# wjwei-handsome/wgatools

Measured on AMD Instinct MI355X. Metric: paf_cigar_ops_per_s (paf2maf+stat), higher is better.
Workload: dtype u8

## Files before the change

wgatools_amd/csrc/wga_kernels_k2s.h:

```cpp
#ifndef WGA_KERNELS_K2S_H
#define WGA_KERNELS_K2S_H

#include "wga_kernels.h"

#define WGA_S_FIFO 320u
#define WGA_S_MAX_JOB_TILES 32u
#define WGA_S_U 4u
#define WGA_S_WAVE_BYTES ((WGA_S_FIFO + 4u) * 8u + 1024u + 1024u + 256u + 272u + 16u)
#ifndef WGA_AUTO_LONG_VARIANT
#define WGA_AUTO_LONG_VARIANT 3
#endif

__global__ __launch_bounds__(256) void k_pseudo_rec_desc(u32 n, const wga_class_sums* sums, const u8* strand_neg, const u64* q_src_off,
                                                         const u64* q_src_len, const u64* skip, const u64* dst_off, const u64* op_off,
                                                         u64 q_fa_bytes, wga_rec_desc* out, u8* tile_flag) {
  const u32 r = blockIdx.x * 256u + threadIdx.x;
  if (r >= n) return;
  const wga_class_sums cs = sums[r];
  wga_rec_desc d;
  d.t_row_off = 0;
  d.q_row_off = dst_off[r] - skip[r];
  d.t_src_off = 0;
  d.t_src_len = skip[r];
  d.q_src_off = q_src_off ? q_src_off[r] : 0ull;
  d.q_src_len = q_src_len ? q_src_len[r] : 0ull;
  d.I_total = cs.i + cs.s;
  d.D_total = cs.d;
  d.L = cs.mx + cs.d;
  const bool clean = !q_src_len || d.q_src_len == cs.mx + cs.i + cs.s;
  const bool inside = !q_src_off || (d.q_src_off >= 32ull && d.q_src_off + d.q_src_len + 32ull <= q_fa_bytes);
  d.neg = (strand_neg[r] != 0 ? 1u : 0u) | (clean ? 0u : 8u);
  out[r] = d;
  if (clean && inside) return;
  const u64 a = op_off[r], b = op_off[r + 1];
  if (b <= a) return;
  for (u64 t = a / WGA_TILE; t <= (b - 1) / WGA_TILE; t++) tile_flag[t] = 1;
}

__device__ __forceinline__ u32 comp4s(u32 x, u32* bad) {
  const u32 sel = x & 0x07070707u;
  const u32 fold = byte_perm(0x474EFF54u, 0x43FF41FFu, sel);
  const u32 comp = byte_perm(0x434E0D41u, 0x47FF54FFu, sel);
  *bad = (x & 0xDFDFDFDFu) ^ fold;
  return comp | (x & 0x20202020u);
}

#define WGA_S_NOINLINE __forceinline__
__device__ WGA_S_NOINLINE void stream_store_bytes(u8* p, u32 o0, u32 o1, u32 o2, u32 o3, int lo, int hi) {
#pragma clang loop vectorize(disable) unroll(disable)
  for (int j = lo; j < hi; j++) {
    const u32 wj = j < 4 ? o0 : j < 8 ? o1 : j < 12 ? o2 : o3;
    p[j] = (u8)(wj >> (8 * (j & 3)));
  }
}
__device__ WGA_S_NOINLINE void stream_report_bad(u64* bad_base_pos, u32 b0, u32 b1, u32 b2, u32 b3, int lo, int hi, u32 Cl,
                                                 i64 Kseg, const u32* fifo, u32 k, u32 nf, u32 adj) {
#pragma clang loop vectorize(disable) unroll(disable)
  for (int j = lo; j < hi; j++) {
    const u32 bw = j < 4 ? b0 : j < 8 ? b1 : j < 12 ? b2 : b3;
    if (((bw >> (8 * (j & 3))) & 0xFFu) == 0u) continue;
    const u32 cj = Cl + (u32)j;
    u32 ad = adj;
    if (fifo) {
      u32 i = k - 1u;
      while (i + 1u < nf && (int)(fifo[2u * (i + 1u)] - cj) <= 0) i++;
      ad = fifo[2u * (i + 1u) + 1u];
    }
    atomicMin(bad_base_pos, (u64)((i64)(u64)(cj - ad) + Kseg));
  }
}

#define WGA_S_PSEUDO 2
#define WGA_S_SYMBOL 3
template <int MODE>
__device__ __forceinline__ u32 stream_glen(u32 c0, u32 c1) {
  return MODE == WGA_S_SYMBOL ? (c1 >> 1) - (c0 >> 1) : MODE == WGA_S_PSEUDO ? ((int)(c1 - c0) > 0 ? c1 - c0 : 0u) : c1 - c0;
}
__device__ __forceinline__ u32 stream_symbol(u32 cu) { return (cu & 1u) ? 0x2D2D2D2Du : 0x30303030u; }
template <int MODE>
__device__ __forceinline__ void stream_row(const ExpandArgs& a, u8* const lds, const u32 lane, const u64 job, const u64 t0,
                                           const u64 t1) {
  const u32 skipm = WGA_RO32(a.job_skip + job);
  u32* const s_fifo = (u32*)lds;
  u32x4_a16* const s_P = (u32x4_a16*)(s_fifo + 2u * (WGA_S_FIFO + 4u));
  u32* const s_q = (u32*)(s_P + 64);
  u32* const s_T = s_q + 256;
  u32x4_a16* const s_lm = (u32x4_a16*)(s_T + 64);
  u64* const s_k = (u64*)(s_lm + 17);
  if (lane < 17u) {
    u32x4_a16 m;
    for (int d = 0; d < 4; d++) m[d] = bytemask(0, (int)lane - 4 * d);
    s_lm[lane] = m;
  }
  constexpr bool QROW = MODE != 0;
  constexpr bool TCOORD = MODE >= WGA_S_PSEUDO;
  constexpr bool SYM = MODE == WGA_S_SYMBOL;
  constexpr u32 COL_MASK = TCOORD ? 0x585u : 0x787u;
  constexpr u32 GAP_MASK = MODE == 0 ? 0x202u : SYM ? 0x504u : 0x404u;
  constexpr u32 SKIP_MASK = MODE == WGA_S_PSEUDO ? 0x212u : 0u;
  const u8* const fa = QROW ? a.q_fa : a.t_fa;
  const u64 fa_bytes = QROW ? a.q_fa_bytes : a.t_fa_bytes;
  const u64 job_lo = t0 * WGA_TILE;
  const u32 q_end = WGA_UNI32((u32)((t1 * WGA_TILE < a.n_ops ? t1 * WGA_TILE : a.n_ops) - job_lo));
  const BufRsrc obuf = buf_make(a.ops + job_lo, (u32)(((a.n_ops - job_lo) < 0x3FFFFFFFull ? (a.n_ops - job_lo) : 0x3FFFFFFFull) * 4ull));

  u32 C_known = 0, cum_known = 0;
  u32 nf = 1;
  u32 e0 = 1;
  u32 pos = 0;
  u32 q = 0;
  u32 q_lo = 0, q_hi = 0;
  u32 rec = 0, re = 0;
  u8* dst_seg = nullptr;
  BufRsrc sbuf = buf_make(fa, 0u);
  u32 S32 = 0;
  bool rc = false;
  bool live = false;
  bool bnd = false;
  bool fin = false;
  u32 C_b = 0, cum_b = 0;
  u32 C_min = 0;
  u64 t = t0;
  u32 ow[4] = {0, 0, 0, 0}, xl0 = 0, xg0 = 0;
  u32 own[4] = {0, 0, 0, 0};

  auto fifo_dedupe = [&]() {
    WGA_WAVE_SYNC();
    u32 n_new = nf;
    if (lane == 0u) {
      u32 w = e0;
      for (u32 r = e0; r < nf; r++) {
        const u32 gs = s_fifo[2u * r], cu = s_fifo[2u * r + 1u];
        const bool dup = w > e0 && s_fifo[2u * (w - 1u)] == gs && (int)(cu - s_fifo[2u * (w - 1u) + 1u]) <= 0 &&
                         (int)(s_fifo[2u * (r + 1u) + 1u] - cu) <= 0;
        if (!dup) {
          s_fifo[2u * w] = gs;
          s_fifo[2u * w + 1u] = cu;
          w++;
        }
      }
      for (u32 k = 0; k < 3u; k++) {
        s_fifo[2u * (w + k)] = s_fifo[2u * (nf + k)];
        s_fifo[2u * (w + k) + 1u] = s_fifo[2u * (nf + k) + 1u];
      }
      n_new = w;
    }
    nf = wave_get_u32(n_new, 0);
    WGA_WAVE_SYNC();
  };

  for (;;) {
    {
      const u32 lim = bnd ? C_b : C_known;
      const bool all = bnd || fin;
      while ((int)(lim - pos) > 0) {
        if (TCOORD && (int)(C_min - pos) > 0) {
          const u32 to = (int)(lim - C_min) > 0 ? C_min : lim;
          u32 c;
          do {
            const u32 idx = e0 + lane < nf ? e0 + lane : nf;
            c = (u32)__popcll(__ballot(idx < nf && (int)(s_fifo[2u * idx] - to) < 0));
            e0 += c;
          } while (c == 64u);
          pos = to;
          continue;
        }
        u8* const A = dst_seg + pos;
        const u32 mis = (u32)(u64)A & 1023u;
        u8* const B = A - mis;
        const u32 room = WGA_S_U * 1024u - mis;
        if (!all && (lim - pos) < room) break;
        const u32 Cs = pos;
        u32 Ce = (lim - pos) < room ? lim : pos + room;
        const u32 Cl0 = Cs - mis;
        if (e0 + 255u < nf) {
          const u32 g255 = WGA_UNI32(s_fifo[2u * (e0 + 255u)]);
          if ((int)(g255 - Ce) < 0) Ce = Cl0 + ((g255 - Cl0) & ~15u);
          if (MODE == WGA_S_PSEUDO && (int)(Ce - Cs) < 16) {
            fifo_dedupe();
            continue;
          }
        }

        s_T[lane] = 0u;
        WGA_WAVE_SYNC();
        u32 nE = 0;
        {
          u32 base = e0, c;
          do {
            const u32 idx = base + lane < nf ? base + lane : nf;
            const u32 gsr = s_fifo[2u * idx] - Cl0;
            const bool in = gsr < Ce - Cl0;
            c = (u32)__popcll(__ballot(in));
            if (in) atomicAdd(&s_T[(gsr >> 4) & 63u], 1u << (8u * (gsr >> 10)));
            base += c;
            nE += c;
          } while (c == 64u);
        }
        WGA_WAVE_SYNC();
        const u32 tw = s_T[lane];
        WGA_WAVE_SYNC();
        const u32 tinc = wave_incl_scan_u32(tw);
        const u32 texc = tinc - tw;
        const u32 ttot = wave_last_u32(tinc);

        u32 kbase = e0;
        u32 qn = 0, rpk = 0, cls = 0;
        u32 adjv[WGA_S_U];
        const u32 wsp = Ce - Cs - 16u, asp = Ce - Cs + 15u;
        const bool any16 = (Ce - Cs) >= 16u;
        u32 qcum = 0;
#pragma unroll
        for (u32 u = 0; u < WGA_S_U; u++) {
          const u32 cnt = (tw >> (8u * u)) & 255u;
          const u32 k = kbase + ((texc >> (8u * u)) & 255u);
          kbase += (ttot >> (8u * u)) & 255u;
          const u32 Cl = Cl0 + 1024u * u + 16u * lane;
          const bool whole = any16 && (Cl - Cs) <= wsp, active = (Cl + 15u - Cs) < asp;
          const u32x4_a1 fe = *(const u32x4_a1*)(s_fifo + 2u * (k - 1u));
          const int rel0 = (int)(fe[0] + stream_glen<MODE>(fe[1], fe[3]) - Cl);
          const bool quiet = whole && cnt == 0u;
          const bool plain = quiet && rel0 <= 0;
          const bool dashes = quiet && rel0 >= 16;
          const bool flagged = active && !(plain || dashes);
          adjv[u] = fe[3];
          cls |= ((plain ? 1u : 0u) | (dashes ? 2u : 0u) | (flagged ? 4u : 0u) | (SYM ? (fe[1] & 1u) << 3 : 0u)) << (4u * u);
          const u64 m = __ballot(flagged);
          if (flagged) {
            const u32 r = qn + lane_rank(m, lane);
            s_q[r & 255u] = (k << 8) | (u << 6) | lane;
            rpk |= (r & 255u) << (8u * u);
          }
          qcum |= (qn > 255u ? 255u : qn) << (8u * u);
          qn += (u32)__popcll(m);
        }
        if (qn > 64u) {
          u32 keep = 1u;
#pragma unroll
          for (u32 u = 2; u <= WGA_S_U; u++) {
            const u32 upto = u == WGA_S_U ? qn : (qcum >> (8u * u)) & 255u;
            const bool sat = u < WGA_S_U && ((qcum >> (8u * u)) & 255u) == 255u;
            if (upto <= 64u && !sat) keep = u;
          }
          const u32 Cn = Cl0 + 1024u * keep;
          if ((int)(Cn - Ce) < 0) Ce = Cn;
          qn = keep == WGA_S_U ? qn : (qcum >> (8u * keep)) & 255u;
          nE = 0;
#pragma unroll
          for (u32 u = 0; u < WGA_S_U; u++)
            if (u < keep) nE += (ttot >> (8u * u)) & 255u;
        }
        const BufRsrc dbuf = buf_make(B, WGA_S_U * 1024u);

        WGA_WAVE_SYNC();
        if (lane < qn) {
          const u32 ent = s_q[lane];
          const u32 k = ent >> 8, Cl = Cl0 + 16u * (ent & 255u);
          int lo = (int)(Cs - Cl), hi = (int)(Ce - Cl);
          lo = lo < 0 ? 0 : (lo > 16 ? 16 : lo);
          hi = hi > 16 ? 16 : (hi < 0 ? 0 : hi);
          const u32x4_a1 ea = *(const u32x4_a1*)(s_fifo + 2u * (k - 1u));
          const u32x4_a1 eb = *(const u32x4_a1*)(s_fifo + 2u * (k + 1u));
          const u32 gs0 = ea[0], cu0 = ea[1], gs1 = ea[2], cu1 = ea[3], gs2 = eb[0], cu2 = eb[1];
          int a1 = (int)(gs0 + stream_glen<MODE>(cu0, cu1) - Cl);
          a1 = a1 < lo ? lo : (a1 > hi ? hi : a1);
          int b1 = (int)(gs1 - Cl);
          b1 = b1 < a1 ? a1 : (b1 > hi ? hi : b1);
          const u32 gl1 = stream_glen<MODE>(cu1, cu2);
          int e1 = gl1 >= 16u ? 16 : b1 + (int)gl1;
          e1 = e1 > hi ? hi : e1;
          bool more = (int)(gs2 - Cl) < hi;
          u32 W0[4], W1[4];
          if (!SYM) {
            buf_load16(sbuf, b1 > a1 ? (rc ? S32 - Cl + cu1 : S32 + Cl - cu1) : WGA_BUF_OOB, W0);
            buf_load16(sbuf, hi > e1 ? (rc ? S32 - Cl + cu2 : S32 + Cl - cu2) : WGA_BUF_OOB, W1);
          }
          const u32x4_a16 La = s_lm[a1], Lb = s_lm[b1], Le = s_lm[e1];
          u32 o[4], bad[4] = {0u, 0u, 0u, 0u};
#pragma unroll
          for (int d = 0; d < 4; d++) {
            if (SYM) {
              o[d] = bfi_b32(La[d], stream_symbol(cu0), bfi_b32(Le[d] & ~Lb[d], stream_symbol(cu1), 0x31313131u));
              continue;
            }
            u32 cp;
            if (rc)
              cp = comp4s(bfi_b32(Lb[d], bswap32(W0[3 - d]), bswap32(W1[3 - d])), &bad[d]);
            else
              cp = bfi_b32(Lb[d], W0[d], W1[d]);
            const u32 md = La[d] | (Le[d] & ~Lb[d]);
            o[d] = bfi_b32(md, 0x2D2D2D2Du, cp);
            bad[d] &= ~md;
          }
          u32 ie = k + 1u;
          while (more) {
            const u32 gsi = s_fifo[2u * ie], cui = s_fifo[2u * ie + 1u], gsn = s_fifo[2u * ie + 2u], cun = s_fifo[2u * ie + 3u];
            const int b = (int)(gsi - Cl);
            const u32 len = stream_glen<MODE>(cui, cun);
            const int e = len >= (u32)(hi - b) ? hi : b + (int)len;
            u32 W[4];
            if (SYM)
              W[0] = W[1] = W[2] = W[3] = 0x31313131u;
            else
              buf_load16(sbuf, rc ? S32 - Cl + cun : S32 + Cl - cun, W);
            const u32x4_a16 Mb = s_lm[b], Me = s_lm[e];
#pragma unroll
            for (int d = 0; d < 4; d++) {
              u32 x = W[d], bw = 0u;
              if (rc) x = comp4s(bswap32(W[3 - d]), &bw);
              if (SYM)
                o[d] = bfi_b32(Mb[d], o[d], bfi_b32(Me[d], stream_symbol(cui), x));
              else
                o[d] = bfi_b32(Mb[d], o[d], bfi_b32(Me[d], 0x2D2D2D2Du, x));
              bad[d] = (bad[d] & Mb[d]) | (bw & ~Me[d]);
            }
            ie++;
            more = (int)(gsn - Cl) < hi;
          }
          if (rc && (bad[0] | bad[1] | bad[2] | bad[3]) != 0u)
            stream_report_bad((u64*)&a.diag[rec].bad_base_pos, bad[0], bad[1], bad[2], bad[3], lo, hi, Cl, (i64)s_k[0], s_fifo, k, nf, 0u);
          const u32x4_a16 ov = {o[0], o[1], o[2], o[3]};
          s_P[lane] = ov;
        }
        WGA_WAVE_SYNC();

        u32 dat[WGA_S_U][4];
        const u32 wsp2 = Ce - Cs - 16u;
#pragma unroll
        for (u32 u = 0; u < WGA_S_U; u++) {
          const u32 Cl = Cl0 + 1024u * u + 16u * lane;
          const u32 c = (cls >> (4u * u)) & 15u;
          if (SYM) {
            dat[u][0] = dat[u][1] = dat[u][2] = dat[u][3] = (c & 2u) ? ((c & 8u) ? 0x2D2D2D2Du : 0x30303030u) : 0x31313131u;
            continue;
          }
          dat[u][0] = dat[u][1] = dat[u][2] = dat[u][3] = (c & 2u) ? 0x2D2D2D2Du : 0u;
          if ((c & 1u) && (int)(Cl - Ce) < 0) buf_load16(sbuf, rc ? S32 - Cl + adjv[u] : S32 + Cl - adjv[u], dat[u]);
        }
        if (rc) {
#pragma unroll
          for (u32 u = 0; u < WGA_S_U; u++) {
            u32 bad[4], x[4];
#pragma unroll
            for (int d = 0; d < 4; d++) x[d] = comp4s(bswap32(dat[u][3 - d]), &bad[d]);
#pragma unroll
            for (int d = 0; d < 4; d++) dat[u][d] = x[d];
            const u32 Cl = Cl0 + 1024u * u + 16u * lane;
            const bool pb = ((cls >> (4u * u)) & 1u) != 0u && (int)(Cl - Ce) < 0 && (bad[0] | bad[1] | bad[2] | bad[3]) != 0u;
            if (__ballot(pb)) {
              if (pb)
                stream_report_bad((u64*)&a.diag[rec].bad_base_pos, bad[0], bad[1], bad[2], bad[3], 0, 16, Cl, (i64)s_k[0], nullptr, 0u, 0u,
                                  adjv[u]);
            }
          }
        }
#pragma unroll
        for (u32 u = 0; u < WGA_S_U; u++) {
          const u32 Cl = Cl0 + 1024u * u + 16u * lane;
          const bool queued = ((cls >> (4u * u)) & 4u) != 0u && (int)(Cl - Ce) < 0;
          if (queued) {
            const u32x4_a16 pv = s_P[(rpk >> (8u * u)) & 255u];
            dat[u][0] = pv[0];
            dat[u][1] = pv[1];
            dat[u][2] = pv[2];
            dat[u][3] = pv[3];
          }
          const bool whole = (Ce - Cs) >= 16u && (Cl - Cs) <= wsp2;
          buf_store16_stream(dbuf, whole ? 1024u * u + 16u * lane : WGA_BUF_OOB, dat[u]);
          if (queued && !whole) {
            int lo = (int)(Cs - Cl), hi = (int)(Ce - Cl);
            lo = lo < 0 ? 0 : lo;
            hi = hi > 16 ? 16 : hi;
            stream_store_bytes(B + 1024u * u + lane * 16u, dat[u][0], dat[u][1], dat[u][2], dat[u][3], lo, hi);
          }
        }
        WGA_WAVE_SYNC();
        e0 += nE;
        pos = Ce;
      }
      fin = false;
    }

    if (bnd || !live) {
      const bool sw = bnd;
      u64 row_off, src_off, src_len, x_a, sb;
      bool neg;
      u32 C_a, cum_a;
      if (bnd) {
        const u64 bnd_op = job_lo + re;
        u64 ren, skip = 0;
        wga_u64x2 src;
        u32 negw;
        do {
          rec++;
          const wga_rec_desc* const rd = a.recs + rec;
          ren = WGA_RO64(a.op_off + rec + 1);
          row_off = WGA_RO64(QROW ? &rd->q_row_off : &rd->t_row_off);
          src = wga_ro16(QROW ? &rd->q_src_off : &rd->t_src_off);
          negw = WGA_RO32((const u32*)&rd->neg);
          if (TCOORD) skip = WGA_RO64(&rd->t_src_len);
          WGA_RO_HERE4(ren, row_off, src.x, src.y);
          WGA_RO_HERE2(negw, skip);
        } while (ren <= bnd_op);
        re = ren - job_lo > (u64)q_end ? q_end : (u32)(ren - job_lo);
        src_off = src.x;
        src_len = src.y;
        neg = (negw & 1u) != 0u;
        x_a = 0;
        sb = 0;
        C_a = C_b;
        cum_a = cum_b;
        if (TCOORD)
          C_min = C_a + (u32)(skip < 0x40000000ull ? skip : 0x40000000ull);
      } else {
        while (t < t1 && ((skipm >> (u32)(t - t0)) & 1u)) t++;
        if (t >= t1) break;
        const wga_tile_desc* const td = a.tdesc + t;
        const u64 tile_start = t * WGA_TILE;
        q = (u32)(tile_start - job_lo);
        WGA_WAVE_SYNC();
        C_known = cum_known = 0u;
        pos = 0u;
        nf = 1u;
        e0 = 1u;
        if (lane < 4u) {
          s_fifo[2u * lane] = 0u;
          s_fifo[2u * lane + 1u] = 0u;
        }
        rec = WGA_RO32(&td->rec);
        const u64 ren = WGA_RO64(&td->re), rs = WGA_RO64(&td->rs);
        const u64 d_mx = WGA_RO64(&td->b_mx), d_i = WGA_RO64(&td->b_i), d_d = WGA_RO64(&td->b_d);
        row_off = WGA_RO64(QROW ? &td->q_row_off : &td->t_row_off);
        src_off = WGA_RO64(QROW ? &td->q_src_off : &td->t_src_off);
        src_len = WGA_RO64(QROW ? &td->q_src_len : &td->t_src_len);
        neg = (WGA_RO32(&td->neg) & 1u) != 0u;
        const u64 skip = TCOORD ? WGA_RO64(&td->t_src_len) : 0ull;
        re = ren - job_lo > (u64)q_end ? q_end : (u32)(ren - job_lo);
        const bool cont = rs < tile_start;
        const u64 b_mx = cont ? d_mx : 0ull, b_i = cont ? d_i : 0ull, b_d = cont ? d_d : 0ull;
        x_a = TCOORD ? b_mx + b_d : b_mx + b_i + b_d;
        sb = QROW ? b_mx + b_i : b_mx + b_d;
        C_a = cum_a = 0u;
        if (TCOORD) {
          const u64 ahead = skip > x_a ? skip - x_a : 0ull;
          C_min = (u32)(ahead < 0x40000000ull ? ahead : 0x40000000ull);
        }
        buf_load16(obuf, q * 4u + lane * 16u, own);
        live = true;
      }
      dst_seg = (u8*)((u64)a.out + row_off + x_a - (u64)C_a);
      rc = QROW && !SYM && neg;
      const u32 adv = C_a - cum_a;
      u64 base;
      if (rc) {
        const u64 top = src_off + src_len;
        const u64 hiB = top > sb ? top - sb : 0ull;
        base = hiB > 0x60000000ull ? hiB - 0x60000000ull : 0ull;
        S32 = (u32)(top - base) - 16u - (u32)sb + adv;
      } else {
        const u64 loB = src_off + sb;
        base = loB > 64ull ? loB - 64ull : 0ull;
        S32 = (u32)(loB - base) - adv;
      }
      base = base > fa_bytes ? fa_bytes : base;
      {
        const u64 left = fa_bytes - base;
        sbuf = buf_make(fa + base, left > 0xFFFFFFF0ull ? 0xFFFFFFF0u : (u32)left);
      }
      if (lane == 0u) s_k[0] = (u64)((i64)sb - (i64)(u64)adv);
      WGA_WAVE_SYNC();
      bnd = false;
      if (sw && re < q_hi) {
        const u32 kb = re - q_lo, e = kb & 3u;
        u32 vl = xl0, vg = xg0;
#pragma unroll
        for (u32 i = 0; i < 3u; i++) {
          const bool valid = q_lo + 4u * lane + i < q_hi && i < e;
          const u32 len = valid ? ow[i] >> 4 : 0u, code = ow[i] & 15u;
          vl += len & bit_mask(COL_MASK, code);
          vg += (len & bit_mask(GAP_MASK, code)) - (len & bit_mask(SKIP_MASK, code));
        }
        C_b = wave_get_u32_dyn(vl, kb >> 2);
        cum_b = wave_get_u32_dyn(vg, kb >> 2);
        bnd = true;
      }
      continue;
    }

    if (q >= q_end) {
      if (pos != C_known) {
        fin = true;
        continue;
      }
      break;
    }
    if ((q & (WGA_TILE - 1u)) == 0u) {
      t = (job_lo + q) / WGA_TILE;
      if ((skipm >> (u32)(t - t0)) & 1u) {
        if (pos != C_known) {
          fin = true;
          continue;
        }
        live = false;
        t++;
        continue;
      }
    }
    if (e0 > 1u) {
      const u32 from = e0 - 1u, count = nf + 3u - from;
      for (u32 i0 = 0; i0 < count; i0 += 64u) {
        const u32 i = i0 + lane;
        u64 v = 0;
        if (i < count) v = *(const u64*)(s_fifo + 2u * (from + i));
        WGA_WAVE_SYNC();
        if (i < count) *(u64*)(s_fifo + 2u * i) = v;
        WGA_WAVE_SYNC();
      }
      nf -= from;
      e0 = 1u;
    }
    if (nf + 256u > WGA_S_FIFO) {
      fin = true;
      if (pos != C_known) continue;
      fin = false;
      if (MODE == WGA_S_PSEUDO) {
        fifo_dedupe();
        if (nf + 256u > WGA_S_FIFO) break;
      }
    }
    q_lo = q;
    q_hi = q + 256u < q_end ? q + 256u : q_end;
    q = q_hi;
    ow[0] = own[0], ow[1] = own[1], ow[2] = own[2], ow[3] = own[3];
    buf_load16(obuf, q_hi < q_end ? q_hi * 4u + lane * 16u : WGA_BUF_OOB, own);
    u32 l[4], g[4], sl = 0, sg = 0, sc = 0;
#pragma unroll
    for (int e = 0; e < 4; e++) {
      const bool valid = q_lo + 4u * lane + (u32)e < q_hi;
      const u32 len = valid ? ow[e] >> 4 : 0u, code = ow[e] & 15u;
      l[e] = len & bit_mask(COL_MASK, code);
      g[e] = (len & bit_mask(GAP_MASK, code)) - (len & bit_mask(SKIP_MASK, code));
      sl += l[e];
      sg += g[e];
      sc += g[e] != 0u ? 1u : 0u;
    }
    const u32 il = wave_incl_scan_u32(sl), ig = wave_incl_scan_u32(sg), ic = wave_incl_scan_u32(sc);
    xl0 = C_known + il - sl;
    xg0 = cum_known + ig - sg;
    {
      u32 xl = xl0, xg = xg0, xc = nf + ic - sc;
#pragma unroll
      for (int e = 0; e < 4; e++) {
        if (g[e] != 0u) {
          s_fifo[2u * xc] = xl;
          s_fifo[2u * xc + 1u] = SYM ? (xg << 1) | (bit_mask(0x404u, ow[e] & 15u) & 1u) : xg;
          xc++;
          xg += g[e];
        }
        xl += l[e];
      }
    }
    C_known += wave_last_u32(il);
    cum_known += wave_last_u32(ig);
    nf += wave_last_u32(ic);
    if (lane < 3u) {
      s_fifo[2u * (nf + lane)] = C_known;
      s_fifo[2u * (nf + lane) + 1u] = SYM ? cum_known << 1 : cum_known;
    }
    WGA_WAVE_SYNC();
    if (re < q_hi) {
      const u32 kb = re - q_lo, e = kb & 3u;
      u32 vl = xl0, vg = xg0;
#pragma unroll
      for (u32 i = 0; i < 3u; i++) {
        const bool valid = q_lo + 4u * lane + i < q_hi && i < e;
        const u32 len = valid ? ow[i] >> 4 : 0u, code = ow[i] & 15u;
        vl += len & bit_mask(COL_MASK, code);
        vg += (len & bit_mask(GAP_MASK, code)) - (len & bit_mask(SKIP_MASK, code));
      }
      C_b = wave_get_u32_dyn(vl, kb >> 2);
      cum_b = wave_get_u32_dyn(vg, kb >> 2);
      bnd = true;
    }
  }
}

__device__ __forceinline__ u64 xcd_job_of_block() {
  const u32 nb = gridDim.x, b = blockIdx.x, x = b & 7u, q = nb >> 3, r = nb & 7u;
  return (u64)(x * q + (x < r ? x : r) + (b >> 3));
}

__device__ __forceinline__ void expand_stream(const ExpandArgs& a) {
  __shared__ u32x4_a16 s_mem[2u * WGA_S_WAVE_BYTES / 16u];
  const u32 lane = threadIdx.x & 63u, wave = WGA_WAVE_ID(threadIdx.x);
  const u64 nt = (a.n_ops + WGA_TILE - 1) / WGA_TILE;
  const u64 job = xcd_job_of_block();
  const u64 t0 = job * a.job_tiles;
  if (t0 >= nt) return;
  const u64 t1 = t0 + a.job_tiles < nt ? t0 + a.job_tiles : nt;
  u8* const lds = (u8*)s_mem + wave * WGA_S_WAVE_BYTES;
  if (wave == 0u)
    stream_row<0>(a, lds, lane, job, t0, t1);
  else
    stream_row<1>(a, lds, lane, job, t0, t1);
}
template <int MODE>
__device__ __forceinline__ void pseudo_stream(const ExpandArgs& a) {
  __shared__ u32x4_a16 s_mem[2u * WGA_S_WAVE_BYTES / 16u];
  const u32 lane = threadIdx.x & 63u, wave = WGA_WAVE_ID(threadIdx.x);
  const u64 nt = (a.n_ops + WGA_TILE - 1) / WGA_TILE;
  const u64 job = 2u * xcd_job_of_block() + wave;
  const u64 t0 = job * a.job_tiles;
  if (t0 >= nt) return;
  const u64 t1 = t0 + a.job_tiles < nt ? t0 + a.job_tiles : nt;
  stream_row<MODE>(a, (u8*)s_mem + wave * WGA_S_WAVE_BYTES, lane, job, t0, t1);
}
#ifndef WGA_S_WAVES_PER_SIMD
#define WGA_S_WAVES_PER_SIMD 5
#endif
__global__ __launch_bounds__(128, WGA_S_WAVES_PER_SIMD) void k_paf2maf_expand_s(ExpandArgs a) { expand_stream(a); }
__global__ __launch_bounds__(128, WGA_S_WAVES_PER_SIMD) void k_pafpseudo_stream(ExpandArgs a) { pseudo_stream<WGA_S_PSEUDO>(a); }
#ifndef WGA_S_SYM_WAVES
#define WGA_S_SYM_WAVES 5
#endif
__global__ __launch_bounds__(128, WGA_S_SYM_WAVES) void k_pafpseudo_stream_sym(ExpandArgs a) { pseudo_stream<WGA_S_SYMBOL>(a); }

#endif
```

Before: 80.08 billion.

## Double-buffer CIGAR op prefetch through LDS via direct DMA loads

Replaces the register-held next-chunk op prefetch with a two-slot LDS ring filled by LDS-direct DMA loads, falling back to buffer loads at the tail. Boundary computation now reads the op words from LDS rather than from per-lane registers. The aim is to lower register pressure and overlap op fetch with the sequence-copy work, and explicit vm_wait calls order the data. In exchange it uses 2 KB more LDS per wave, which may lower occupancy, and adds waits that can serialize on outstanding sequence loads.

```diff
diff --git a/wgatools_amd/csrc/wga_kernels_k2s.h b/wgatools_amd/csrc/wga_kernels_k2s.h
--- a/wgatools_amd/csrc/wga_kernels_k2s.h
+++ b/wgatools_amd/csrc/wga_kernels_k2s.h
@@ -6,7 +6,7 @@
 #define WGA_S_FIFO 320u
 #define WGA_S_MAX_JOB_TILES 32u
 #define WGA_S_U 4u
-#define WGA_S_WAVE_BYTES ((WGA_S_FIFO + 4u) * 8u + 1024u + 1024u + 256u + 272u + 16u)
+#define WGA_S_WAVE_BYTES ((WGA_S_FIFO + 4u) * 8u + 1024u + 1024u + 256u + 272u + 16u + 2u * 1024u)
 #ifndef WGA_AUTO_LONG_VARIANT
 #define WGA_AUTO_LONG_VARIANT 3
 #endif
@@ -87,6 +87,7 @@
   u32* const s_T = s_q + 256;
   u32x4_a16* const s_lm = (u32x4_a16*)(s_T + 64);
   u64* const s_k = (u64*)(s_lm + 17);
+  u32x4_a16* const s_ops = (u32x4_a16*)(s_k + 2);
   if (lane < 17u) {
     u32x4_a16 m;
     for (int d = 0; d < 4; d++) m[d] = bytemask(0, (int)lane - 4 * d);
@@ -121,8 +122,37 @@
   u32 C_b = 0, cum_b = 0;
   u32 C_min = 0;
   u64 t = t0;
-  u32 ow[4] = {0, 0, 0, 0}, xl0 = 0, xg0 = 0;
-  u32 own[4] = {0, 0, 0, 0};
+  u32 xl0 = 0, xg0 = 0;
+  u32 cur = 1;
+  bool landed = true;
+  auto ops_request = [&](const u32 qq, const u32 slot) {
+    const u32 o = qq + 4u * lane;
+    u32x4_a16* const dstp = s_ops + 64u * slot;
+    WGA_WAVE_SYNC();
+    if (o + 4u <= q_end) {
+      lds_dma16_after_reads(a.ops + job_lo, o * 4u, dstp);
+    } else if (o < q_end) {
+      u32 w[4];
+      buf_load16(obuf, o * 4u, w);
+      const u32x4_a16 wv = {w[0], w[1], w[2], w[3]};
+      dstp[lane] = wv;
+    }
+    landed = false;
+  };
+  auto boundary = [&]() {
+    const u32 kb = re - q_lo, bl = kb >> 2, e = kb & 3u;
+    const u32x4_a16 w = s_ops[64u * cur + bl];
+    u32 vl = wave_get_u32_dyn(xl0, bl), vg = wave_get_u32_dyn(xg0, bl);
+#pragma unroll
+    for (u32 i = 0; i < 3u; i++) {
+      const u32 len = i < e ? w[i] >> 4 : 0u, code = w[i] & 15u;
+      vl += len & bit_mask(COL_MASK, code);
+      vg += (len & bit_mask(GAP_MASK, code)) - (len & bit_mask(SKIP_MASK, code));
+    }
+    C_b = WGA_UNI32(vl);
+    cum_b = WGA_UNI32(vg);
+    bnd = true;
+  };
 
   auto fifo_dedupe = [&]() {
     WGA_WAVE_SYNC();
@@ -336,6 +366,10 @@
           }
           dat[u][0] = dat[u][1] = dat[u][2] = dat[u][3] = (c & 2u) ? 0x2D2D2D2Du : 0u;
           if ((c & 1u) && (int)(Cl - Ce) < 0) buf_load16(sbuf, rc ? S32 - Cl + adjv[u] : S32 + Cl - adjv[u], dat[u]);
+        }
+        if (!SYM || !landed) {
+          vm_wait(0);
+          landed = true;
         }
         if (rc) {
 #pragma unroll
@@ -445,7 +479,9 @@
           const u64 ahead = skip > x_a ? skip - x_a : 0ull;
           C_min = (u32)(ahead < 0x40000000ull ? ahead : 0x40000000ull);
         }
-        buf_load16(obuf, q * 4u + lane * 16u, own);
+        if (!landed) vm_wait(0);
+        cur = 1u;
+        ops_request(q, 0u);
         live = true;
       }
       dst_seg = (u8*)((u64)a.out + row_off + x_a - (u64)C_a);
@@ -470,20 +506,7 @@
       if (lane == 0u) s_k[0] = (u64)((i64)sb - (i64)(u64)adv);
       WGA_WAVE_SYNC();
       bnd = false;
-      if (sw && re < q_hi) {
-        const u32 kb = re - q_lo, e = kb & 3u;
-        u32 vl = xl0, vg = xg0;
-#pragma unroll
-        for (u32 i = 0; i < 3u; i++) {
-          const bool valid = q_lo + 4u * lane + i < q_hi && i < e;
-          const u32 len = valid ? ow[i] >> 4 : 0u, code = ow[i] & 15u;
-          vl += len & bit_mask(COL_MASK, code);
-          vg += (len & bit_mask(GAP_MASK, code)) - (len & bit_mask(SKIP_MASK, code));
-        }
-        C_b = wave_get_u32_dyn(vl, kb >> 2);
-        cum_b = wave_get_u32_dyn(vg, kb >> 2);
-        bnd = true;
-      }
+      if (sw && re < q_hi) boundary();
       continue;
     }
 
@@ -531,8 +554,13 @@
     q_lo = q;
     q_hi = q + 256u < q_end ? q + 256u : q_end;
     q = q_hi;
-    ow[0] = own[0], ow[1] = own[1], ow[2] = own[2], ow[3] = own[3];
-    buf_load16(obuf, q_hi < q_end ? q_hi * 4u + lane * 16u : WGA_BUF_OOB, own);
+    cur ^= 1u;
+    if (!landed) {
+      vm_wait(0);
+      landed = true;
+    }
+    const u32x4_a16 ow = s_ops[64u * cur + lane];
+    if (q_hi < q_end) ops_request(q_hi, cur ^ 1u);
     u32 l[4], g[4], sl = 0, sg = 0, sc = 0;
 #pragma unroll
     for (int e = 0; e < 4; e++) {
@@ -568,21 +596,9 @@
       s_fifo[2u * (nf + lane) + 1u] = SYM ? cum_known << 1 : cum_known;
     }
     WGA_WAVE_SYNC();
-    if (re < q_hi) {
-      const u32 kb = re - q_lo, e = kb & 3u;
-      u32 vl = xl0, vg = xg0;
-#pragma unroll
-      for (u32 i = 0; i < 3u; i++) {
-        const bool valid = q_lo + 4u * lane + i < q_hi && i < e;
-        const u32 len = valid ? ow[i] >> 4 : 0u, code = ow[i] & 15u;
-        vl += len & bit_mask(COL_MASK, code);
-        vg += (len & bit_mask(GAP_MASK, code)) - (len & bit_mask(SKIP_MASK, code));
-      }
-      C_b = wave_get_u32_dyn(vl, kb >> 2);
-      cum_b = wave_get_u32_dyn(vg, kb >> 2);
-      bnd = true;
-    }
+    if (re < q_hi) boundary();
   }
+  if (!landed) vm_wait(0);
 }
 
 __device__ __forceinline__ u64 xcd_job_of_block() {
```

Result: no change. 81.14 billion, median of 6 (+1.3%).
